# DassHydro-dev/smash

Measured on AMD Instinct MI355X. Metric: cell-timesteps/s, forward+adjoint sweep, higher is better.
Workload: dtype f32

## Files before the change

smash_amd/csrc/smashx.hip:

```cpp
#include "../../include/smashx.h"

#include <hip/hip_runtime.h>
#include <rccl/rccl.h>

#include <dlfcn.h>

#include <algorithm>
#include <cstdio>
#include <cstdlib>
#include <cstring>
#include <string>
#include <vector>

#include "sx_cost.h"
#include "sx_jreg.h"
#include "sx_kernels.h"
#include "sx_ensemble.h"
#include "sx_interception.h"
#include "sx_meanforcing.h"
#include "sx_prcpindices.h"
#include "sx_plan.h"
#include "sx_selftest.h"

namespace {
// ... 279 lines not shown
struct PeerSeg { int rank, first, count; };

struct Launch { hipEvent_t a, b; int kind; double cellsteps; };

}

struct smashx_plan {
    smashx_config cfg{};
    SxSchedule sch;
    int n = 0, npad = 0, nt = 0, ng = 0, st = 0;
    long n2 = 0;
    int M = 0;
    int Tc = 0, nchunks = 0;
    bool have_forcing = false, have_options = false, have_qobs = false, uploaded = false;
    bool chunk_ready = false, adj_ready = false;
    smashx_options opt{};
    std::vector<float> wgauge;
    hipStream_t stream = nullptr;
    hipStream_t stream_r = nullptr;
    int Tp = 0;
    bool hi_tape = true;
    int chain_from = 1;
    bool chain_stage = false; SxStageTables stg{}; int stg_blocks = 0, stg_rows_extra = 0; size_t stg_lds = 0;
    size_t vlds_fwd = 0, vlds_adj = 0;
    std::vector<hipEvent_t> buf_free;
    std::vector<double> round_ncells;
    bool chain_used = false;
    bool chain = true;
    int n_out = 0, n_in = 0;
    int *d_out_x = nullptr, *d_in_x = nullptr;
    float *halo_out = nullptr, *halo_in = nullptr;
    smashx_halo_fn halo_fn = nullptr; void* halo_user = nullptr;
    SxComm* xcomm = nullptr;
    std::vector<PeerSeg> out_segs, in_segs;
    int *d_out_xp = nullptr, *d_in_xp = nullptr;
    float *x_out = nullptr, *x_in = nullptr;
    float* x_keep = nullptr; size_t x_keep_cap = 0;
    std::vector<void*> allocs; std::vector<size_t> alloc_bytes;
    double bytes = 0;
    double hbm_free_at_plan = -1.0, hbm_total = -1.0;
    SxDeviceArrays A{};
    int* d_cell_flat = nullptr;
    int* d_sparse_idx = nullptr;
    float last_jobs_d = 0.f, last_jreg_d = 0.f;
    long n_sparse = 0;
    float* d_stage = nullptr;
// ... 94 lines not shown
    hipStream_t cur = nullptr;
    void mark_begin(int kind, hipStream_t st, double cellsteps = 0.0) {
        cur = st; Launch l; l.a = event(); l.b = nullptr; l.kind = kind; l.cellsteps = cellsteps;
        if (l.a) (void)hipEventRecord(l.a, st);
        launches.push_back(l);
    }
    void mark_end() { Launch& l = launches.back(); l.b = event(); if (l.b) (void)hipEventRecord(l.b, cur); }
};

namespace {

int set_device(const smashx_plan* p) {
    if (p->cfg.device >= 0) HIPCHK(hipSetDevice(p->cfg.device));
    return 0;
}

int sublevels_env() {
    const char* e = getenv("SMASHX_SUBLEVELS");
    const char* e0 = getenv("SMASHX_SUBLEVELS_R0");
    return (e ? std::max(1, atoi(e)) : 1) | ((e0 ? std::max(1, atoi(e0)) : 1) << 8);
}

int chunk_len(const smashx_plan* p, int c) { return std::min(p->Tc, p->nt - c * p->Tc); }

int ensure_chunk_buffers(smashx_plan* p, bool adjoint) {
    const int st = p->st;
    const bool has_hi = (st == 2 || st == 3);
    const double ntape_full = (st == 5 ? 3.0 : st == 3 ? 4.0 : st == 2 ? 3.0 : 2.0);
    const double ntape_lean = has_hi ? ntape_full - 1.0 + 1.0 / SX_HIK : ntape_full;
    double ntape = ntape_full;
    if (!p->chunk_ready) {
        if ((p->n_out > 0 || p->n_in > 0) && p->cfg.chunk_steps <= 0)
            return fail(SMASHX_E_ARG, "a tile with boundary series needs an explicit chunk_steps (identical on every rank; pipe_steps = 0 then means no sub-chunks)");
        const int nt16 = (p->nt + 15) / 16 * 16;
        int Tc = p->cfg.chunk_steps > 0 ? (p->cfg.chunk_steps + 15) / 16 * 16 : 0;
        {
            size_t fr = 0, tot = 0;
            HIPCHK(hipMemGetInfo(&fr, &tot));
            p->hbm_free_at_plan = (double)fr; p->hbm_total = (double)tot;
        }
        if (Tc == 0) {
            size_t fr = 0, tot = 0;
            HIPCHK(hipMemGetInfo(&fr, &tot));
            const double avail = (double)fr * 0.85 - 1.0e9;
            auto fit = [&](double nt_) { return (long)(avail / (4.0 * ((double)p->npad * (2 + nt_) + (double)std::max(p->sch.nxslots, 1)))) / 16 * 16; };
            long t = fit(ntape_full);
            if (has_hi && t < nt16) {
                const long tl = fit(ntape_lean);
                auto nch = [&](long tc) { tc = std::max<long>(16, std::min<long>(nt16, tc)); return (double)((p->nt + tc - 1) / tc); };
                if (0.67 * (1.0 / nch(tl) - 1.0 / nch(t)) > 0.14) { p->hi_tape = false; t = tl; }
            }
            Tc = (int)std::max<long>(16, std::min<long>(nt16, t));
        }
        if (const char* e = getenv("SMASHX_HI_TAPE")) p->hi_tape = atoi(e) != 0;
        if (!has_hi) p->hi_tape = true;
        ntape = p->hi_tape ? ntape_full : ntape_lean;
        (void)ntape;
        Tc = std::min(Tc, nt16);
        {
            const int nch = (p->nt + Tc - 1) / Tc;
            Tc = std::min(Tc, ((p->nt + nch - 1) / nch + 15) / 16 * 16);
        }
        p->Tc = Tc;
        p->A.Tc = Tc;
        p->A.nx = std::max(p->sch.nxslots, 1);
        p->nchunks = (p->nt + Tc - 1) / Tc;
        {
            int want = p->cfg.pipe_steps > 0 ? p->cfg.pipe_steps : Tc;
            const int nsub = std::max(1, (Tc + want / 2) / want);
            p->Tp = std::min(Tc, ((Tc + nsub - 1) / nsub + 15) / 16 * 16);
        }
        int rc;
        if ((rc = p->dmalloc(&p->A.qtT, (size_t)p->npad * Tc))) return rc;
        if ((rc = p->dmalloc(&p->A.xT, (size_t)std::max(p->sch.nxslots, 1) * Tc))) return rc;
        HIPCHK(hipMemsetAsync(p->A.qtT, 0, (size_t)p->npad * Tc * 4, p->stream));
        HIPCHK(hipMemsetAsync(p->A.xT, 0, (size_t)std::max(p->sch.nxslots, 1) * Tc * 4, p->stream));
        p->chunk_ready = true;
    }
    if (p->h_qsim_domain && !p->A.qdT) {
        int rc;
        if ((rc = p->dmalloc(&p->A.qdT, (size_t)p->npad * p->Tc))) return rc;
    }
    if (adjoint && !p->adj_ready) {
        int rc;
        const size_t cs = (size_t)p->npad * p->Tc;
        if (p->A.qsk) { p->dfree(p->A.qsk); p->A.qsk = nullptr; }
        {
            const size_t extra = (size_t)p->sch.max_stage * p->npad * 4;
            const double ntp = 3.0 + ((st == 5 || ((st == 2 || st == 3) && p->hi_tape)) ? 1.0 : (st == 2 || st == 3) ? 1.0 / SX_HIK : 0.0) + (st == 3 ? 1.0 : 0.0);
            size_t fr = 0, tot = 0;
            HIPCHK(hipMemGetInfo(&fr, &tot));
            const double need = 4.0 * ((double)cs * ntp + (double)extra + (double)p->npad * (14 + (p->nchunks > 1 ? 5.0 * p->nchunks : 0.0))
                                       + 2.0 * (double)std::max(p->ngc, 1) * p->nt) + 3.0e9;
            const char* e = getenv("SMASHX_HR_SKEW");
            p->A.hr_skew = (e ? atoi(e) != 0 : true) && (double)fr > need;
            if ((rc = p->dmalloc(&p->A.hrT, cs + (p->A.hr_skew ? extra : 0)))) return rc;
        }
        if ((rc = p->dmalloc(&p->A.tape_hp, cs))) return rc;
        if ((rc = p->dmalloc(&p->A.tape_hft, cs))) return rc;
        if (st == 5 || ((st == 2 || st == 3) && p->hi_tape)) { if ((rc = p->dmalloc(&p->A.tape_hi, cs))) return rc; }
        else if (st == 2 || st == 3) { if ((rc = p->dmalloc(&p->A.ckpt_hi, cs / SX_HIK))) return rc; }
        if (st == 3) { if ((rc = p->dmalloc(&p->A.tape_hst, cs))) return rc; }
        if (p->nchunks > 1) { if ((rc = p->dmalloc(&p->ckpt, (size_t)p->nchunks * 5 * p->npad))) return rc; }
        float** g[14] = {&p->A.ci_b, &p->A.cp_b, &p->A.cft_b, &p->A.cst_b, &p->A.exc_b, &p->A.lr_b,
                         &p->A.hi_b, &p->A.hp_b, &p->A.hft_b, &p->A.hst_b, &p->A.hlr_b, &p->A.px_b[0], &p->A.px_b[1], &p->A.px_b[2]};
        for (auto q : g) if ((rc = p->dmalloc(q, (size_t)p->npad))) return rc;
        if ((rc = p->dmalloc(&p->A.qgb, (size_t)std::max(p->ngc, 1) * p->nt))) return rc;
        if ((rc = p->dmalloc(&p->d_qsim_b, (size_t)std::max(p->ng, 1) * p->nt))) return rc;
        p->adj_ready = true;
    }
    if (p->A.ncs > 0 && !p->A.qsk) {
        const size_t need = (size_t)p->A.ncs * 16 * ((size_t)p->Tc / 4 + p->stg_rows_extra + 1);
        size_t fr = 0, tot = 0;
        HIPCHK(hipMemGetInfo(&fr, &tot));
        if ((double)fr > (double)need + 2.0e9) { int rc; if ((rc = p->dmalloc(&p->A.qsk, need / 4))) return rc; }
    }
    return 0;
}

SxDeviceArrays view_at(const smashx_plan* p, int off) {
    SxDeviceArrays B = p->A;
    B.k0 = 0; B.k1 = p->n;
    const size_t q = (size_t)(off / 4);
    B.qtT = p->A.qtT + q * p->npad * 4;
    if (p->A.hrT) B.hrT = p->A.hrT + q * p->npad * 4;
    if (p->A.qdT) B.qdT = p->A.qdT + q * p->npad * 4;
    if (!p->chain) B.qsk = nullptr;
    B.xT = p->A.xT + q * p->A.nx * 4;
    if (p->A.qtdT) B.qtdT = p->A.qtdT + q * p->npad * 4;
    if (p->A.xdT) B.xdT = p->A.xdT + q * p->A.nx * 4;
    if (p->A.tape_hp) B.tape_hp = p->A.tape_hp + (size_t)off * p->npad;
    if (p->A.tape_hft) B.tape_hft = p->A.tape_hft + (size_t)off * p->npad;
    if (p->A.tape_hi) B.tape_hi = p->A.tape_hi + (size_t)off * p->npad;
    if (p->A.ckpt_hi) B.ckpt_hi = p->A.ckpt_hi + (size_t)(off / SX_HIK) * p->npad;
    if (p->A.tape_hst) B.tape_hst = p->A.tape_hst + (size_t)off * p->npad;
    return B;
}

template <int ST>
void launch_vert_fwd(smashx_plan* p, const SxDeviceArrays& B, bool tape, int t0, int T) {
    const dim3 grid((B.k1 - B.k0 + SX_VBLOCK - 1) / SX_VBLOCK), block(SX_VBLOCK);
    p->mark_begin(0, p->stream, (double)(B.k1 - B.k0) * T);
    const bool cf = B.prcp16 != nullptr;
    const size_t vl = p->vlds_fwd;
    if (tape) { if (cf) hipLaunchKernelGGL((sx_k_vert_fwd<ST, true, true>), grid, block, vl, p->stream, B, t0, T);
                else    hipLaunchKernelGGL((sx_k_vert_fwd<ST, true, false>), grid, block, vl, p->stream, B, t0, T); }
    else      { if (cf) hipLaunchKernelGGL((sx_k_vert_fwd<ST, false, true>), grid, block, vl, p->stream, B, t0, T);
                else    hipLaunchKernelGGL((sx_k_vert_fwd<ST, false, false>), grid, block, vl, p->stream, B, t0, T); }
// ... 48 lines not shown
    return c;
}
int chain_first(const smashx_plan* p) {
    const int nr = p->sch.nrounds;
    return (p->chain && nr - p->chain_from >= 2) ? p->chain_from : nr;
}
void reset_chain_counters(smashx_plan* p, hipStream_t st) {
    (void)hipMemsetAsync(p->A.prog, 0, (size_t)p->sch.ngroups * sizeof(int), st);
    (void)hipMemsetAsync(p->A.prog + p->sch.ngroups + 1, 0, sizeof(int), st);
}
void route_fwd_rounds(smashx_plan* p, int off, bool tape, int t0, int T, hipStream_t st) {
    SxDeviceArrays B = view_at(p, off);
    if (!p->dom_q_active) B.qdT = nullptr;
    const size_t lds = (size_t)2 * p->M * sizeof(float4);
    const int cf = chain_first(p);
    for (int r = 0; r < cf; ++r) {
        const int g0 = p->sch.round_group_begin[r], ngr = p->sch.round_group_begin[r + 1] - g0;
        p->mark_begin(1, st, round_cells(p, r, r + 1) * T);
        if (tape) hipLaunchKernelGGL((sx_k_route_fwd<true, false>), dim3(ngr), dim3(p->M), lds, st, B, g0, g0 + ngr, t0, T);
        else      hipLaunchKernelGGL((sx_k_route_fwd<false, false>), dim3(ngr), dim3(p->M), lds, st, B, g0, g0 + ngr, t0, T);
        p->mark_end();
    }
}
bool route_fwd_chained(smashx_plan* p, int off, bool tape, int t0, int T, hipStream_t st, hipEvent_t inputs_read = nullptr) {
    const int nr = p->sch.nrounds, cf = chain_first(p);
    if (cf >= nr) return false;
    SxDeviceArrays B = view_at(p, off);
    if (!p->dom_q_active) B.qdT = nullptr;
    const size_t lds = (size_t)2 * p->M * sizeof(float4);
    const int g0 = p->sch.round_group_begin[cf], g1 = p->sch.ngroups;
    reset_chain_counters(p, st);
    const int grid = g1 - g0;
    p->mark_begin(5, st, round_cells(p, cf, nr) * T);
    if (B.qsk)
        hipLaunchKernelGGL((sx_k_chain_transpose<true>), dim3((p->stg_blocks + SX_STG_WAVES - 1) / SX_STG_WAVES), dim3(64 * SX_STG_WAVES), p->stg_lds * SX_STG_WAVES, st, B, p->stg, g0, (T + SX_BT - 1) / SX_BT, p->stg_blocks, (int)p->stg_lds);
    const bool early = B.qsk && inputs_read && !B.qdT;
    if (early) (void)hipEventRecord(inputs_read, st);
    if (tape) hipLaunchKernelGGL((sx_k_route_fwd<true, true>), dim3(grid), dim3(p->M), lds, st, B, g0, g1, t0, T);
    else      hipLaunchKernelGGL((sx_k_route_fwd<false, true>), dim3(grid), dim3(p->M), lds, st, B, g0, g1, t0, T);
    p->mark_end();
    p->chain_used = true;
    return early;
}
bool route_fwd(smashx_plan* p, int off, bool tape, int t0, int T, hipEvent_t inputs_read = nullptr) {
    route_fwd_rounds(p, off, tape, t0, T, p->stream_r);
    return route_fwd_chained(p, off, tape, t0, T, p->stream_r, inputs_read);
}
void route_adj_chained(smashx_plan* p, int off, int t0, int T, hipStream_t st) {
    const int nr = p->sch.nrounds, cf = chain_first(p);
    if (cf >= nr) return;
    const SxDeviceArrays B = view_at(p, off);
    const size_t lds = (size_t)2 * p->M * sizeof(float4);
    const int g0 = p->sch.round_group_begin[cf], g1 = p->sch.ngroups;
    reset_chain_counters(p, st);
    const int grid = g1 - g0;
    p->mark_begin(6, st, round_cells(p, cf, nr) * T);
    hipLaunchKernelGGL((sx_k_route_adj<true>), dim3(grid), dim3(p->M), lds, st, B, g0, g1, t0, T);
    if (B.qsk)
        hipLaunchKernelGGL((sx_k_chain_transpose<false>), dim3((p->stg_blocks + SX_STG_WAVES - 1) / SX_STG_WAVES), dim3(64 * SX_STG_WAVES), p->stg_lds * SX_STG_WAVES, st, B, p->stg, g0, (T + SX_BT - 1) / SX_BT, p->stg_blocks, (int)p->stg_lds);
    p->mark_end();
    p->chain_used = true;
}
void route_adj_rounds(smashx_plan* p, int off, int t0, int T, hipStream_t st) {
    const SxDeviceArrays B = view_at(p, off);
    const size_t lds = (size_t)2 * p->M * sizeof(float4);
    const int cf = chain_first(p);
    for (int r = cf - 1; r >= 0; --r) {
        const int g0 = p->sch.round_group_begin[r], ngr = p->sch.round_group_begin[r + 1] - g0;
        p->mark_begin(2, st, round_cells(p, r, r + 1) * T);
        hipLaunchKernelGGL((sx_k_route_adj<false>), dim3(ngr), dim3(p->M), lds, st, B, g0, g0 + ngr, t0, T);
        p->mark_end();
    }
}
void route_adj(smashx_plan* p, int off, int t0, int T) {
    route_adj_chained(p, off, t0, T, p->stream_r);
    route_adj_rounds(p, off, t0, T, p->stream_r);
}

SxCostArgs cost_args(smashx_plan* p, float jobs_b) {
    SxCostArgs C{};
    C.ng = p->ng; C.nt = p->nt; C.s0 = p->opt.optimize_start_step - 1; C.njf = p->opt.njf;
    for (int j = 0; j < SX_MAXJF; ++j) { C.jobs_fun[j] = p->opt.jobs_fun[j]; C.wjobs_fun[j] = p->opt.wjobs_fun[j]; }
    C.dt = p->cfg.dt; C.dx = p->cfg.dx;
    C.qg = p->A.qg; C.qgb = p->A.qgb; C.ngc = p->ngc;
    C.gauge_gid = p->d_gauge_gid; C.gauge_flwacc = p->d_gauge_flwacc; C.area = p->d_area; C.wgauge = p->d_wgauge;
    C.qobs = p->d_qobs; C.qsim_b = p->d_qsim_b; C.sums = p->d_sums; C.coef = p->d_coef; C.out = p->d_cost_out;
    C.med = p->d_med; C.med_idx = p->d_med_idx;
    C.nslots = p->med_nslots; C.slot = p->d_med_slot; C.medx = p->d_medx; C.medx_idx = p->d_medx_idx;
    C.jobs_b = jobs_b;
    return C;
}

int run_cost(smashx_plan* p, int adjoint, float cost_b) {
    if (p->ng == 0 && p->med_nslots == 0) return 0;
    SxCostArgs C = cost_args(p, cost_b);
    p->mark_begin(4, p->stream_r);
    if (p->ng > 0) hipLaunchKernelGGL(sx_k_cost_sums, dim3(p->ng), dim3(64), 0, p->stream_r, C);
    if (p->med_nslots > 0) {
        HIPCHK(hipMemsetAsync(p->d_medx, 0, (size_t)p->med_nslots * sizeof(float), p->stream_r));
// ... 719 lines not shown
    const int ns_max = nsub_of(p->Tc);
    const size_t keep_sub = (size_t)std::max(p->n_in, 1) * (size_t)((p->Tp + 3) / 4) * 4;
    const bool keep_in = adjoint && halo && p->n_in > 0 && C > 1;
    if (keep_in && p->x_keep_cap < keep_sub * ns_max * (size_t)(C - 1)) {
        if (p->x_keep) p->dfree(p->x_keep);
        p->x_keep = nullptr; p->x_keep_cap = 0;
        if ((rc = p->dmalloc(&p->x_keep, keep_sub * ns_max * (size_t)(C - 1)))) return rc;
        p->x_keep_cap = keep_sub * ns_max * (size_t)(C - 1);
    }
    auto inlet_series = [&](int c, int jb, int off, int t0, int T, bool recompute, hipStream_t st) -> int {
        float* msg = native ? p->x_in : p->halo_in;
        float* kept = (keep_in && c < C - 1) ? p->x_keep + ((size_t)c * ns_max + jb) * keep_sub : nullptr;
        const size_t bytes = (size_t)p->n_in * (size_t)((T + 3) / 4) * 4 * sizeof(float);
        if (recompute && kept) {
            HIPCHK(hipMemcpyAsync(msg, kept, bytes, hipMemcpyDeviceToDevice, st));
        } else {
            if ((rc = hook(0, t0, T, st))) return rc;
            if (kept) HIPCHK(hipMemcpyAsync(kept, msg, bytes, hipMemcpyDeviceToDevice, st));
        }
        halo_move(false, false, off, T, st);
        return 0;
    };
    static const bool early_release = []() { const char* e = getenv("SMASHX_EARLY_RELEASE"); return !(e && e[0] == '0'); }();
    auto forward_chunk = [&](int c, bool tape, bool recompute = false) -> int {
        const int t0c = c * p->Tc, Tcur = chunk_len(p, c), ns = nsub_of(Tcur);
        std::vector<hipEvent_t> ev(ns);
        auto launch_v = [&](int jb) -> int {
            const int off = jb * p->Tp, T = std::min(p->Tp, Tcur - off);
            if (jb < (int)p->buf_free.size() && p->buf_free[jb]) { HIPCHK(hipStreamWaitEvent(sV, p->buf_free[jb], 0)); p->buf_free[jb] = nullptr; }
            vert_fwd(p, off, tape, t0c + off, T);
            ev[jb] = p->event(); HIPCHK(hipEventRecord(ev[jb], sV));
            return 0;
        };
        for (int jb = 0; jb < ns; ++jb) if ((rc = launch_v(jb))) return rc;
        for (int jb = 0; jb < ns; ++jb) {
            const int off = jb * p->Tp, T = std::min(p->Tp, Tcur - off);
            if (halo && p->n_in > 0 && (rc = inlet_series(c, jb, off, t0c + off, T, recompute, sR))) return rc;
            HIPCHK(hipStreamWaitEvent(sR, ev[jb], 0));
            if ((int)p->buf_free.size() <= jb) p->buf_free.resize(jb + 1, nullptr);
            p->buf_free[jb] = p->event();
            const bool released = route_fwd(p, off, tape, t0c + off, T, early_release ? p->buf_free[jb] : nullptr);
            if (halo && p->n_out > 0 && !recompute) {
                halo_move(true, true, off, T, sR);
                if ((rc = hook(1, t0c + off, T, sR))) return rc;
            }
            if (!released) HIPCHK(hipEventRecord(p->buf_free[jb], sR));
        }
        return 0;
    };
    p->dom_q_active = !adjoint && p->h_qsim_domain && p->A.qdT;
    auto export_domain = [&](int c) -> int {
        const int t0c = c * p->Tc, Tcur = chunk_len(p, c);
        HIPCHK(hipStreamSynchronize(sV));
        HIPCHK(hipStreamSynchronize(sR));
        const long plane = p->dom_sparse ? p->n_sparse : p->n2;
        const int* idx = p->dom_sparse ? p->d_sparse_idx : p->d_cell_flat;
        const int nbmax = (int)std::max<long>(1, std::min<long>(p->stage_planes * p->n2 / plane, 1 << 15));
        for (int which = 0; which < 2; ++which) {
            float* host = which ? p->h_net_prcp_domain : p->h_qsim_domain;
            const float* src = which ? p->A.qtT : p->A.qdT;
            if (!host || !src) continue;
            for (int tl0 = 0; tl0 < Tcur; tl0 += nbmax) {
                const int nb = std::min(nbmax, Tcur - tl0);
                if (!p->dom_sparse || p->tiled)
// ... 22 lines not shown
            }
            if ((rc = forward_chunk(c, c == C - 1))) return rc;
        }
        if ((rc = run_cost(p, 1, cost_b))) return rc;
        {
            float* gv[14] = {p->A.ci_b, p->A.cp_b, p->A.cft_b, p->A.cst_b, p->A.exc_b, p->A.hi_b, p->A.hp_b, p->A.hft_b, p->A.hst_b,
                             p->A.lr_b, p->A.hlr_b, p->A.px_b[0], p->A.px_b[1], p->A.px_b[2]};
            const int ps = p->st;
            auto pfi = [&](int slot) { const int f = param_field(ps, slot); return f; };
            auto sfi = [&](int slot) { const int f = state_field(ps, slot); return f < 0 ? -1 : SMASHX_GNP + f; };
            const int gi[14] = {pfi(0), pfi(1), pfi(2), pfi(3), pfi(4), sfi(0), sfi(1), sfi(2), sfi(3), pfi(5), sfi(4), pfi(6), pfi(7), pfi(8)};
            bool waited[2] = {false, false};
            for (int q = 0; q < 14; ++q) {
                const bool on_r = (q == 9 || q == 10);
                hipStream_t sq = on_r ? sR : sV;
                HIPCHK(hipMemsetAsync(gv[q], 0, (size_t)p->npad * 4, sq));
                if (p->opt.njr > 0 && gi[q] >= 0 && jreg_optim(p, gi[q]) > 0) {
                    if (!waited[on_r ? 1 : 0]) { HIPCHK(hipStreamWaitEvent(sq, p->ev_j, 0)); waited[on_r ? 1 : 0] = true; }
                    hipLaunchKernelGGL(k_gather, dim3((p->n + 255) / 256), dim3(256), 0, sq, gv[q], p->d_jg[gi[q]], p->d_cell_flat, p->n);
                }
            }
        }
        if (p->ng == 0) HIPCHK(hipMemsetAsync(p->A.qgb, 0, (size_t)std::max(p->ngc, 1) * p->nt * 4, sR));
        for (int c = C - 1; c >= 0; --c) {
            const int t0c = c * p->Tc, Tcur = chunk_len(p, c);
            if (C > 1 && c < C - 1) {
                float* src[5];
                for (int i = 0; i < 5; ++i) src[i] = p->ckpt + ((size_t)c * 5 + i) * p->npad;
                if ((rc = restore_states(p, src))) return rc;
                if ((rc = forward_chunk(c, true, true))) return rc;
            }
            const int nsa = (Tcur + p->Tp - 1) / p->Tp;
            for (int jb = nsa - 1; jb >= 0; --jb) {
                const int off = jb * p->Tp, T = std::min(p->Tp, Tcur - off);
                if (halo && p->n_out > 0) {
                    if ((rc = hook(2, t0c + off, T, sR))) return rc;
                    halo_move(false, true, off, T, sR);
                }
                route_adj(p, off, t0c + off, T);
                hipEvent_t e = p->event();
                HIPCHK(hipEventRecord(e, sR));
                HIPCHK(hipStreamWaitEvent(sV, e, 0));
                vert_adj(p, off, t0c + off, T);
                if (halo && p->n_in > 0) {
                    halo_move(true, false, off, T, sR);
                    if ((rc = hook(3, t0c + off, T, sR))) return rc;
                }
            }
        }
    }
    {
        hipEvent_t e = p->event();
        HIPCHK(hipEventRecord(e, sR));
        HIPCHK(hipStreamWaitEvent(sV, e, 0));
    }
    HIPCHK(hipEventRecord(p->ev1, sV));
    HIPCHK(hipStreamSynchronize(sV));
    HIPCHK(hipStreamSynchronize(sR));
    if (p->opt.njr > 0) HIPCHK(hipStreamSynchronize(p->stream_j));
    HIPCHK(hipGetLastError());
    if (p->chain_used) {
        int stalled = 0;
        HIPCHK(hipMemcpy(&stalled, p->A.prog + p->sch.ngroups, sizeof(int), hipMemcpyDeviceToHost));
        if (stalled) {
            if (getenv("SMASHX_VERBOSE")) {
// ... 4 lines not shown
                std::vector<int> pr(p->sch.ngroups);
                (void)hipMemcpy(pr.data(), p->A.prog, pr.size() * sizeof(int), hipMemcpyDeviceToHost);
                for (int g = p->sch.round_group_begin[chain_first(p)]; g < p->sch.ngroups; ++g) fprintf(stderr, " %d", pr[g]);
                fprintf(stderr, " (n_in %d n_out %d)\n", p->n_in, p->n_out);
            }
            *stalled_out = true; return 0;
        }
    }
    smashx_timing& tm = p->timing;
    std::memset(&tm, 0, sizeof(tm));
    (void)hipEventElapsedTime(&tm.sweep_ms, p->ev0, p->ev1);
    for (const Launch& l : p->launches) {
        float ms = 0.f;
        if (l.a && l.b) (void)hipEventElapsedTime(&ms, l.a, l.b);
        switch (l.kind) {
            case 0: tm.vert_fwd_ms += ms; tm.vert_fwd_launches++; tm.cellsteps[0] += l.cellsteps; break;
            case 1: tm.route_fwd_ms += ms; tm.route_fwd_launches++; tm.cellsteps[1] += l.cellsteps; break;
            case 2: tm.route_adj_ms += ms; tm.route_adj_launches++; tm.cellsteps[2] += l.cellsteps; break;
            case 3: tm.vert_adj_ms += ms; tm.vert_adj_launches++; tm.cellsteps[3] += l.cellsteps; break;
            case 5: tm.route_fwd_ms += ms; tm.route_fwd_launches++; tm.cellsteps[1] += l.cellsteps;
                    tm.route_fwd_chained_ms += ms; tm.route_fwd_chained_launches++; break;
            case 6: tm.route_adj_ms += ms; tm.route_adj_launches++; tm.cellsteps[2] += l.cellsteps;
                    tm.route_adj_chained_ms += ms; tm.route_adj_chained_launches++; break;
            default: tm.cost_ms += ms; break;
        }
    }
    tm.n_chunks = p->nchunks; tm.chunk_steps = p->Tc; tm.pipe_steps = p->Tp; tm.n_rounds = p->sch.nrounds; tm.n_groups = p->sch.ngroups;
    tm.device_bytes = p->bytes;
    tm.max_stage = p->sch.max_stage;
    tm.chain_staged = (p->chain && p->A.qsk != nullptr) ? 1 : 0;
    tm.n_chained_groups = chain_first(p) < p->sch.nrounds ? p->sch.ngroups - p->sch.round_group_begin[chain_first(p)] : 0;
    p->last_adjoint = adjoint;
    return 0;
}

int smashx_set_domain_outputs(smashx_plan* p, float* qsim_domain, float* net_prcp_domain, int sparse) {
    if (!p) return fail(SMASHX_E_ARG, "null plan");
    if (sparse && !p->d_sparse_idx && (qsim_domain || net_prcp_domain))
        return fail(SMASHX_E_ARG, "sparse domain outputs need mesh.path (the sparse cell numbering)");
    p->h_qsim_domain = qsim_domain; p->h_net_prcp_domain = net_prcp_domain; p->dom_sparse = sparse ? 1 : 0;
    return 0;
}

int smashx_debug_group_times(smashx_plan* p, long long* out, int* round_of_group) {
    if (!p || !out) return fail(SMASHX_E_ARG, "null argument");
    if (!p->A.gtime) return fail(SMASHX_E_STATE, "group tracing is off (SMASHX_TRACE_GROUPS=1)");
// ... 1189 lines not shown
```

smash_amd/csrc/sx_kernels.h:

```cpp
#pragma once

#include <hip/hip_runtime.h>

#include <climits>

#include "sx_ops.h"
#include "sx_tangent.h"
#include "sx_vic.h"

#define SX_BT 4
#define SX_VBLOCK 256

__device__ __forceinline__ void sx_lds_barrier() {
    __builtin_amdgcn_fence(__ATOMIC_RELEASE, "workgroup", "local");
    __builtin_amdgcn_s_barrier();
    __builtin_amdgcn_fence(__ATOMIC_ACQUIRE, "workgroup", "local");
}

__device__ __forceinline__ void sx_lds_wave_fence() {
    __builtin_amdgcn_fence(__ATOMIC_RELEASE, "workgroup", "local");
    __builtin_amdgcn_wave_barrier();
    __builtin_amdgcn_fence(__ATOMIC_ACQUIRE, "workgroup", "local");
}

// ... 84 lines not shown
    __builtin_amdgcn_fence(__ATOMIC_ACQUIRE, "agent");
}
__device__ __forceinline__ void sx_publish(int* prog, int blocks) {
    __builtin_amdgcn_fence(__ATOMIC_RELEASE, "agent");
    __hip_atomic_store((sx_gint*)prog, blocks, __ATOMIC_RELAXED, __HIP_MEMORY_SCOPE_AGENT);
}

struct SxDeviceArrays {
    int n, npad, nt, Tc;
    int k0, k1;
    int nx;
    float dt, dx;
    const float* prcp; const float* pet;
    const unsigned short* prcp16; const float* petd; const float* pet_ratio;
    float prcp_c, prcp_gap; int hour0;
    float *ci, *cp, *cft, *cst, *exc, *lr;
    float* px[3]; float* px_b[3];
    float *rt_a, *rt_f, *rt_denf, *rt_denb;
    int* flwacc;
    float *hi, *hp, *hft, *hst, *hlr;
    float *ci_b, *cp_b, *cft_b, *cst_b, *exc_b, *lr_b, *hi_b, *hp_b, *hft_b, *hst_b, *hlr_b;
    float *qtT, *hrT;
    int hr_skew;
    float *qtdT, *xdT, *qgd;
    float* qdT;
    float *tape_hi, *tape_hp, *tape_hft, *tape_hst;
    float* ckpt_hi;
    float* xT;
    float* qsk; int cs0, ncs;
    float *qg, *qgb;
    int* cell_gauge;
    const int *g_slot_begin, *g_dmax;
    const int *s_cell, *s_stage, *s_sub, *s_wsub, *s_child, *s_ccount, *s_parent, *s_xout;
    const int *x_prod, *x_cons;
    int* prog;
    int ngroups;
    int spin_limit;
    int mute_group;
    long long* gtime;
};

struct SxStageTables {
    const int* wb_slot0; const int* wb_n; const int* wb_smin; const int* wb_spread;
    const int* fifo_g; const int* fifo_s;
};
#ifndef SX_STG_PF
// ... 436 lines not shown
            cell = c;
            const int4 cw = reinterpret_cast<const int4*>(A.s_child)[sb + j];
            ch01 = (unsigned)cw.x; ch23 = (unsigned)cw.y; ch45 = (unsigned)cw.z; ch67 = (unsigned)cw.w;
            ccount = A.s_ccount[sb + j]; xout = A.s_xout[sb + j];
            a = A.rt_a[c]; f = A.rt_f[c]; den = (TAN || DFORM) ? A.rt_denb[c] : A.rt_denf[c]; hlr = TAN ? A.hlr_b[c] : A.hlr[c];
            if (TAN) { const float lrv = A.lr[c]; ad = a * ((A.dt / (60.f * lrv)) * A.lr_b[c] / lrv); }
            hasup = A.flwacc[c] > 1;
            gid = A.cell_gauge[c];
        } else {
            xin = -1 - c;
        }
    }
    const float dt = A.dt, dx = A.dx;
    const SxDiv dden = sx_mkdiv(den), ddt = sx_mkdiv(dt);
    const int* wprog = nullptr;
    int seen = 0;
    if (CHAIN && xin >= 0) { const int pg = A.x_prod[xin]; if (pg >= g0 && pg < gend) wprog = A.prog + pg; }
    const bool staged = CHAIN && !TAN && A.qsk != nullptr && valid && !wprog;
    const float4* src = staged ? reinterpret_cast<const float4*>(A.qsk) + (size_t)stage * A.ncs + (sb + j - A.cs0)
                      : (cell >= 0) ? reinterpret_cast<const float4*>(TAN ? A.qtdT : A.qtT) + cell
                                    : reinterpret_cast<const float4*>(TAN ? A.xdT : A.xT) + (xin >= 0 ? xin : 0);
    const size_t sstride = staged ? (size_t)A.ncs : (cell >= 0) ? (size_t)A.npad : (size_t)A.nx;
    float4* x4 = reinterpret_cast<float4*>(TAN ? A.xdT : A.xT);
    float4* hr4 = reinterpret_cast<float4*>(A.hrT);
    const int hs = A.hr_skew ? stage : 0;
    float* gauge_out = TAN ? A.qgd : A.qg;
    const float4 zero4 = make_float4(0.f, 0.f, 0.f, 0.f);
    auto fetch = [&](int tb) -> float4 { return cell >= 0 ? sx_gload4s(src + (size_t)tb * sstride) : sx_gload4(src + (size_t)tb * sstride); };

    float4 nxt[MU], outq[MU], outh[MU], nhr[MU];
    if (CHAIN && wprog) sx_wait_prog(wprog, min(MU - stage, nb), seen, SX_PROG_STALL(A), A.spin_limit, g);
#pragma unroll
    for (int u = 0; u < MU; ++u) {
        const int tb = u - stage;
        nxt[u] = (valid && tb >= 0 && tb < nb) ? fetch(tb) : zero4;
        nhr[u] = (TAN && valid && cell >= 0 && tb >= 0 && tb < nb) ? sx_gload4(hr4 + (size_t)(tb + hs) * A.npad + cell) : zero4;
        outq[u] = zero4; outh[u] = zero4;
    }
    const int nsuper = nb + dmax;
    const int nmacro = (nsuper + MU - 1) / MU;
    for (int mw = 0; mw <= nmacro; ++mw) {
        float4 cur[MU], chr[MU];
#pragma unroll
        for (int u = 0; u < MU; ++u) { cur[u] = nxt[u]; sx_pin(cur[u]); if (TAN) { chr[u] = nhr[u]; sx_pin(chr[u]); } }
        if (CHAIN) asm volatile("s_waitcnt vmcnt(0)" ::: "memory");
        if (mw > 0 && cell >= 0) {
#pragma unroll
            for (int u = 0; u < MU; ++u) {
                const int tb = MU * (mw - 1) + u - stage;
                if (tb >= 0 && tb < nb) {
                    if (xout >= 0) x4[(size_t)tb * A.nx + xout] = outq[u];
                    if (TAPE) sx_gstore4s(hr4 + (size_t)(tb + hs) * A.npad + cell, outh[u]);
                    if (A.qdT) reinterpret_cast<float4*>(A.qdT)[(size_t)tb * A.npad + cell] = outq[u];
                    if (gid >= 0) {
                        const float qv[4] = {outq[u].x, outq[u].y, outq[u].z, outq[u].w};
#pragma unroll
                        for (int i = 0; i < SX_BT; ++i)
                            if (tb * SX_BT + i < T) gauge_out[(size_t)gid * A.nt + t0 + tb * SX_BT + i] = qv[i];
                    }
                }
            }
        }
        if (mw == nmacro) break;
        if (CHAIN && wprog) sx_wait_prog(wprog, min(MU * (mw + 2) - stage, nb), seen, SX_PROG_STALL(A), A.spin_limit, g);
#pragma unroll
        for (int u = 0; u < MU; ++u) {
            const int tb = MU * (mw + 1) + u - stage;
            nxt[u] = (valid && tb >= 0 && tb < nb) ? fetch(tb) : zero4;
            if (TAN) nhr[u] = (valid && cell >= 0 && tb >= 0 && tb < nb) ? sx_gload4(hr4 + (size_t)(tb + hs) * A.npad + cell) : zero4;
        }
#pragma unroll
        for (int u = 0; u < MU; ++u) {
            const int w = MU * mw + u;
            const int tb = w - stage;
            const bool act = valid && tb >= 0 && tb < nb;
            float4* pub = sx_lds + (size_t)(w & 1) * M;
            auto child_val = [&](unsigned e) -> float4 {
                const float4* row = sx_lds + (size_t)((w + 1 + (int)((e >> 15) & 1u)) & 1) * M;
                return row[min((int)(e & 0x7fffu), M - 1)];
            };
          auto sub_pass = [&](const int sl) {
            if (act && sub == sl) {
                const int tl = tb * SX_BT;
                if (cell >= 0) {
                    float s[SX_BT];
                    {
                        const float4 v0 = child_val(ch01 & 0xffffu), v1 = child_val(ch01 >> 16);
                        const bool h0 = ccount > 0, h1 = ccount > 1;
                        s[0] = (h0 ? v0.x : 0.f) + (h1 ? v1.x : 0.f); s[1] = (h0 ? v0.y : 0.f) + (h1 ? v1.y : 0.f);
                        s[2] = (h0 ? v0.z : 0.f) + (h1 ? v1.z : 0.f); s[3] = (h0 ? v0.w : 0.f) + (h1 ? v1.w : 0.f);
                    }
                    for (int c = 2; c < ccount; ++c) {
                        const unsigned wd = c < 4 ? ch23 : c < 6 ? ch45 : ch67;
// ... 97 lines not shown
    bool hasup = false;
    const int nsubw = __builtin_amdgcn_readfirstlane(m > 0 ? A.s_wsub[sb + min(j, m - 1)] : 1);
    if (valid && A.s_cell[sb + j] == INT_MIN) valid = false;
    if (valid) {
        const int c = A.s_cell[sb + j];
        rstage = dmax - A.s_stage[sb + j];
        sub = A.s_sub[sb + j];
        par = A.s_parent[sb + j];
        if (par >= 0) { psame = (par & 0x40000000) != 0; par &= 0xffff; }
        if (c >= 0) {
            cell = c;
            xout = A.s_xout[sb + j];
            a = A.rt_a[c]; f = A.rt_f[c]; den = A.rt_denb[c]; lr = A.lr[c];
            hr_b = A.hlr_b[c]; lr_b = A.lr_b[c];
            hasup = A.flwacc[c] > 1;
            gid = A.cell_gauge[c];
        } else {
            xin = -1 - c;
        }
    }
    const float dt = A.dt, dx = A.dx;
    const SxDiv dden = sx_mkdiv(den), ddt = sx_mkdiv(dt), dlr = sx_mkdiv((lr * lr) * 60.f);
    float4* x4 = reinterpret_cast<float4*>(A.xT);
    const float4* hr4p = reinterpret_cast<const float4*>(A.hrT);
    const int hs = A.hr_skew ? dmax - rstage : 0;
    float4* qt4 = reinterpret_cast<float4*>(A.qtT);
    const float4 zero4 = make_float4(0.f, 0.f, 0.f, 0.f);
    const bool root_in = (cell >= 0 && par < 0 && xout >= 0);
    const bool staged = CHAIN && A.qsk != nullptr && valid && (cell >= 0 || (xin >= 0 && !(A.x_prod[xin] >= g0 && A.x_prod[xin] < gend)));
    float4* const dst = staged ? reinterpret_cast<float4*>(A.qsk) + (size_t)(dmax - rstage) * A.ncs + (sb + j - A.cs0)
                               : (cell >= 0) ? qt4 + cell : x4 + (xin >= 0 ? xin : 0);
    const size_t dstride = staged ? (size_t)A.ncs : (cell >= 0) ? (size_t)A.npad : (size_t)A.nx;

    const float* seedp = (gid >= 0) ? A.qgb + (size_t)gid * A.nt + t0 : nullptr;
    auto load_seed = [&](int tb) -> float4 {
        float4 v = make_float4(0.f, 0.f, 0.f, 0.f);
        if (gid >= 0) {
            const int tl = tb * SX_BT;
            if (tl + 0 < T) v.x = sx_gload1(seedp + tl + 0);
            if (tl + 1 < T) v.y = sx_gload1(seedp + tl + 1);
            if (tl + 2 < T) v.z = sx_gload1(seedp + tl + 2);
            if (tl + 3 < T) v.w = sx_gload1(seedp + tl + 3);
        }
        return v;
    };
    const int* wprog = nullptr;
    int seen = 0;
    if (CHAIN && root_in) { const int cg = A.x_cons[xout]; if (cg >= g0 && cg < gend) wprog = A.prog + cg; }
    auto fetch_in = [&](int tb) -> float4 { return sx_gload4(x4 + (size_t)tb * A.nx + xout); };
    float4 nhr[MU], nin[MU], nsd[MU], outq[MU];
    if (CHAIN && wprog) sx_wait_prog(wprog, min(MU - rstage, nb), seen, SX_PROG_STALL(A), A.spin_limit, g);
#pragma unroll
    for (int u = 0; u < MU; ++u) {
        const int tbr = u - rstage;
        const int tb = nb - 1 - tbr;
        const bool ok = valid && tbr >= 0 && tbr < nb;
        nhr[u] = (ok && cell >= 0) ? sx_gload4s(hr4p + (size_t)(tb + hs) * A.npad + cell) : zero4;
        nin[u] = (ok && root_in) ? fetch_in(tb) : zero4;
        nsd[u] = ok ? load_seed(tb) : zero4;
        outq[u] = zero4;
    }
    const int nsuper = nb + dmax;
    const int nmacro = (nsuper + MU - 1) / MU;
    for (int mw = 0; mw <= nmacro; ++mw) {
        float4 chr[MU], cin[MU], csd[MU];
#pragma unroll
        for (int u = 0; u < MU; ++u) {
            chr[u] = nhr[u]; cin[u] = nin[u]; csd[u] = nsd[u];
            sx_pin(chr[u]); sx_pin(cin[u]); sx_pin(csd[u]);
        }
        if (CHAIN) asm volatile("s_waitcnt vmcnt(0)" ::: "memory");
        if (mw > 0 && valid) {
#pragma unroll
            for (int u = 0; u < MU; ++u) {
                const int tbr = MU * (mw - 1) + u - rstage;
                if (tbr >= 0 && tbr < nb) {
                    const int tb = nb - 1 - tbr;
                    sx_gstore4(dst + (size_t)tb * dstride, outq[u]);
                }
            }
        }
        if (mw == nmacro) break;
        if (CHAIN && wprog) sx_wait_prog(wprog, min(MU * (mw + 2) - rstage, nb), seen, SX_PROG_STALL(A), A.spin_limit, g);
#pragma unroll
        for (int u = 0; u < MU; ++u) {
            const int tbr = MU * (mw + 1) + u - rstage;
            const int tb = nb - 1 - tbr;
            const bool ok = valid && tbr >= 0 && tbr < nb;
            nhr[u] = (ok && cell >= 0) ? sx_gload4s(hr4p + (size_t)(tb + hs) * A.npad + cell) : zero4;
            nin[u] = (ok && root_in) ? fetch_in(tb) : zero4;
            nsd[u] = ok ? load_seed(tb) : zero4;
        }
#pragma unroll
        for (int u = 0; u < MU; ++u) {
            const int w = MU * mw + u;
            const int tbr = w - rstage;
            const bool act = valid && tbr >= 0 && tbr < nb;
            float4* pub = sx_lds + (size_t)(w & 1) * M;
            const float4* prev = sx_lds + (size_t)((w + 1) & 1) * M;
          auto sub_pass = [&](const int sl) {
            if (act && sub == sl) {
                const int tb = nb - 1 - tbr;
                const int tl = tb * SX_BT;
                float4 in4 = cin[u];
                if (par >= 0) in4 = psame ? pub[par] : prev[par];
                if (cell >= 0) {
                    const float hrv[SX_BT] = {chr[u].x, chr[u].y, chr[u].z, chr[u].w};
                    const float inv[SX_BT] = {in4.x, in4.y, in4.z, in4.w};
                    const float sdv[SX_BT] = {csd[u].x, csd[u].y, csd[u].z, csd[u].w};
                    float pb[SX_BT], qtb[SX_BT];
                    float tmpb[SX_BT], qrb[SX_BT], himb[SX_BT], a1b[SX_BT];
                    float nq[SX_BT];
#pragma unroll
                    for (int i = SX_BT - 1; i >= 0; --i) {
                        float q_b = 0.f;
// ... 157 lines not shown
```

Baseline: 54.80 billion.

## Keep chained routing tape per chunk and overlap next chunk's chained adjoint

Adds a persistent per-chunk buffer (hrk) that stores the chained-routing hr tape for every chunk except the last, so the adjoint sweep no longer recomputes the chained forward routing for those chunks. The skewed hr tape becomes a circular row buffer addressed by wrapped row indices instead of extra padded rows, which removes the free-memory check and the extra allocation. The chained adjoint for the previous chunk is also launched early on the routing stream so it overlaps with the vertical adjoint of the current chunk. In exchange it uses extra device memory proportional to the number of chunks, and it adds wrap-around index arithmetic inside the forward and adjoint routing kernels.

Result: faster. 57.68 billion, median of 6 (+5.2%).

```diff
diff --git a/smash_amd/csrc/smashx.hip b/smash_amd/csrc/smashx.hip
--- a/smash_amd/csrc/smashx.hip
+++ b/smash_amd/csrc/smashx.hip
@@ -325,6 +325,7 @@
     bool hi_tape = true;
     int chain_from = 1;
     bool chain_stage = false; SxStageTables stg{}; int stg_blocks = 0, stg_rows_extra = 0; size_t stg_lds = 0;
+    float* hrk = nullptr; bool hrk_tried = false, early_adj = true;
     size_t vlds_fwd = 0, vlds_adj = 0;
     std::vector<hipEvent_t> buf_free;
     std::vector<double> round_ncells;
@@ -465,6 +466,7 @@
 }
 
 int chunk_len(const smashx_plan* p, int c) { return std::min(p->Tc, p->nt - c * p->Tc); }
+int chain_first(const smashx_plan* p);
 
 int ensure_chunk_buffers(smashx_plan* p, bool adjoint) {
     const int st = p->st;
@@ -506,6 +508,7 @@
         }
         p->Tc = Tc;
         p->A.Tc = Tc;
+        p->A.hr_rows = Tc / 4;
         p->A.nx = std::max(p->sch.nxslots, 1);
         p->nchunks = (p->nt + Tc - 1) / Tc;
         {
@@ -529,15 +532,9 @@
         const size_t cs = (size_t)p->npad * p->Tc;
         if (p->A.qsk) { p->dfree(p->A.qsk); p->A.qsk = nullptr; }
         {
-            const size_t extra = (size_t)p->sch.max_stage * p->npad * 4;
-            const double ntp = 3.0 + ((st == 5 || ((st == 2 || st == 3) && p->hi_tape)) ? 1.0 : (st == 2 || st == 3) ? 1.0 / SX_HIK : 0.0) + (st == 3 ? 1.0 : 0.0);
-            size_t fr = 0, tot = 0;
-            HIPCHK(hipMemGetInfo(&fr, &tot));
-            const double need = 4.0 * ((double)cs * ntp + (double)extra + (double)p->npad * (14 + (p->nchunks > 1 ? 5.0 * p->nchunks : 0.0))
-                                       + 2.0 * (double)std::max(p->ngc, 1) * p->nt) + 3.0e9;
             const char* e = getenv("SMASHX_HR_SKEW");
-            p->A.hr_skew = (e ? atoi(e) != 0 : true) && (double)fr > need;
-            if ((rc = p->dmalloc(&p->A.hrT, cs + (p->A.hr_skew ? extra : 0)))) return rc;
+            p->A.hr_skew = e ? atoi(e) != 0 : true;
+            if ((rc = p->dmalloc(&p->A.hrT, cs))) return rc;
         }
         if ((rc = p->dmalloc(&p->A.tape_hp, cs))) return rc;
         if ((rc = p->dmalloc(&p->A.tape_hft, cs))) return rc;
@@ -558,6 +555,23 @@
         HIPCHK(hipMemGetInfo(&fr, &tot));
         if ((double)fr > (double)need + 2.0e9) { int rc; if ((rc = p->dmalloc(&p->A.qsk, need / 4))) return rc; }
     }
+    if (adjoint && !p->hrk_tried) {
+        p->hrk_tried = true;
+        const int cf = chain_first(p);
+        const char* e = getenv("SMASHX_KEEP_CHAIN_TAPE");
+        const bool want = e ? atoi(e) != 0 : true;
+        if (const char* ea = getenv("SMASHX_EARLY_ADJ_CHAIN")) p->early_adj = atoi(ea) != 0;
+        if (want && p->nchunks > 1 && cf < p->sch.nrounds && !p->tiled && p->n_in == 0 && p->n_out == 0 && p->Tp >= p->Tc) {
+            const int kcs0 = p->sch.g_slot_begin[p->sch.round_group_begin[cf]], kncs = p->sch.nslots - kcs0;
+            const size_t need = (size_t)(p->nchunks - 1) * (size_t)(p->Tc / 4) * (size_t)kncs * 16;
+            size_t fr = 0, tot = 0;
+            HIPCHK(hipMemGetInfo(&fr, &tot));
+            if (kncs > 0 && (double)fr > (double)need + 2.0e9) {
+                int rc; if ((rc = p->dmalloc(&p->hrk, need / 4))) return rc;
+                p->A.kcs0 = kcs0; p->A.kncs = kncs;
+            }
+        }
+    }
     return 0;
 }
 
@@ -566,7 +580,8 @@
     B.k0 = 0; B.k1 = p->n;
     const size_t q = (size_t)(off / 4);
     B.qtT = p->A.qtT + q * p->npad * 4;
-    if (p->A.hrT) B.hrT = p->A.hrT + q * p->npad * 4;
+    B.hrk = nullptr;
+    if (p->A.hrT) { if (p->A.hr_skew) B.hr_row0 = (int)q; else B.hrT = p->A.hrT + q * p->npad * 4; }
     if (p->A.qdT) B.qdT = p->A.qdT + q * p->npad * 4;
     if (!p->chain) B.qsk = nullptr;
     B.xT = p->A.xT + q * p->A.nx * 4;
@@ -661,10 +676,11 @@
         p->mark_end();
     }
 }
-bool route_fwd_chained(smashx_plan* p, int off, bool tape, int t0, int T, hipStream_t st, hipEvent_t inputs_read = nullptr) {
+bool route_fwd_chained(smashx_plan* p, int off, bool tape, int t0, int T, hipStream_t st, hipEvent_t inputs_read = nullptr, float* hrk = nullptr) {
     const int nr = p->sch.nrounds, cf = chain_first(p);
     if (cf >= nr) return false;
     SxDeviceArrays B = view_at(p, off);
+    if (hrk) { B.hrk = hrk; B.hr_row0 = 0; tape = true; }
     if (!p->dom_q_active) B.qdT = nullptr;
     const size_t lds = (size_t)2 * p->M * sizeof(float4);
     const int g0 = p->sch.round_group_begin[cf], g1 = p->sch.ngroups;
@@ -681,24 +697,26 @@
     p->chain_used = true;
     return early;
 }
-bool route_fwd(smashx_plan* p, int off, bool tape, int t0, int T, hipEvent_t inputs_read = nullptr) {
-    route_fwd_rounds(p, off, tape, t0, T, p->stream_r);
-    return route_fwd_chained(p, off, tape, t0, T, p->stream_r, inputs_read);
-}
-void route_adj_chained(smashx_plan* p, int off, int t0, int T, hipStream_t st) {
+void route_adj_chained(smashx_plan* p, int off, int t0, int T, hipStream_t st, float* hrk = nullptr, bool launch = true, bool copy = true) {
     const int nr = p->sch.nrounds, cf = chain_first(p);
     if (cf >= nr) return;
-    const SxDeviceArrays B = view_at(p, off);
+    SxDeviceArrays B = view_at(p, off);
+    if (hrk) { B.hrk = hrk; B.hr_row0 = 0; }
     const size_t lds = (size_t)2 * p->M * sizeof(float4);
     const int g0 = p->sch.round_group_begin[cf], g1 = p->sch.ngroups;
-    reset_chain_counters(p, st);
     const int grid = g1 - g0;
-    p->mark_begin(6, st, round_cells(p, cf, nr) * T);
-    hipLaunchKernelGGL((sx_k_route_adj<true>), dim3(grid), dim3(p->M), lds, st, B, g0, g1, t0, T);
-    if (B.qsk)
+    if (launch) {
+        reset_chain_counters(p, st);
+        p->mark_begin(6, st, round_cells(p, cf, nr) * T);
+        hipLaunchKernelGGL((sx_k_route_adj<true>), dim3(grid), dim3(p->M), lds, st, B, g0, g1, t0, T);
+        p->mark_end();
+        p->chain_used = true;
+    }
+    if (copy && B.qsk) {
+        p->mark_begin(7, st);
         hipLaunchKernelGGL((sx_k_chain_transpose<false>), dim3((p->stg_blocks + SX_STG_WAVES - 1) / SX_STG_WAVES), dim3(64 * SX_STG_WAVES), p->stg_lds * SX_STG_WAVES, st, B, p->stg, g0, (T + SX_BT - 1) / SX_BT, p->stg_blocks, (int)p->stg_lds);
-    p->mark_end();
-    p->chain_used = true;
+        p->mark_end();
+    }
 }
 void route_adj_rounds(smashx_plan* p, int off, int t0, int T, hipStream_t st) {
     const SxDeviceArrays B = view_at(p, off);
@@ -710,10 +728,6 @@
         hipLaunchKernelGGL((sx_k_route_adj<false>), dim3(ngr), dim3(p->M), lds, st, B, g0, g0 + ngr, t0, T);
         p->mark_end();
     }
-}
-void route_adj(smashx_plan* p, int off, int t0, int T) {
-    route_adj_chained(p, off, t0, T, p->stream_r);
-    route_adj_rounds(p, off, t0, T, p->stream_r);
 }
 
 SxCostArgs cost_args(smashx_plan* p, float jobs_b) {
@@ -1479,6 +1493,8 @@
         return 0;
     };
     static const bool early_release = []() { const char* e = getenv("SMASHX_EARLY_RELEASE"); return !(e && e[0] == '0'); }();
+    const bool keep = adjoint && C > 1 && p->hrk && !halo && chain_first(p) < p->sch.nrounds;
+    auto kept_rows = [&](int c) -> float* { return (keep && c < C - 1) ? p->hrk + (size_t)c * (size_t)(p->Tc / 4) * (size_t)p->A.kncs * 4 : nullptr; };
     auto forward_chunk = [&](int c, bool tape, bool recompute = false) -> int {
         const int t0c = c * p->Tc, Tcur = chunk_len(p, c), ns = nsub_of(Tcur);
         std::vector<hipEvent_t> ev(ns);
@@ -1496,7 +1512,9 @@
             HIPCHK(hipStreamWaitEvent(sR, ev[jb], 0));
             if ((int)p->buf_free.size() <= jb) p->buf_free.resize(jb + 1, nullptr);
             p->buf_free[jb] = p->event();
-            const bool released = route_fwd(p, off, tape, t0c + off, T, early_release ? p->buf_free[jb] : nullptr);
+            float* const hrk = kept_rows(c);
+            route_fwd_rounds(p, off, tape, t0c + off, T, sR);
+            const bool released = (hrk && recompute) ? false : route_fwd_chained(p, off, tape, t0c + off, T, sR, early_release ? p->buf_free[jb] : nullptr, hrk);
             if (halo && p->n_out > 0 && !recompute) {
                 halo_move(true, true, off, T, sR);
                 if ((rc = hook(1, t0c + off, T, sR))) return rc;
@@ -1565,6 +1583,7 @@
             }
         }
         if (p->ng == 0) HIPCHK(hipMemsetAsync(p->A.qgb, 0, (size_t)std::max(p->ngc, 1) * p->nt * 4, sR));
+        bool adj_queued = false;
         for (int c = C - 1; c >= 0; --c) {
             const int t0c = c * p->Tc, Tcur = chunk_len(p, c);
             if (C > 1 && c < C - 1) {
@@ -1580,10 +1599,16 @@
                     if ((rc = hook(2, t0c + off, T, sR))) return rc;
                     halo_move(false, true, off, T, sR);
                 }
-                route_adj(p, off, t0c + off, T);
+                route_adj_chained(p, off, t0c + off, T, sR, kept_rows(c), !adj_queued, true);
+                adj_queued = false;
+                route_adj_rounds(p, off, t0c + off, T, sR);
                 hipEvent_t e = p->event();
                 HIPCHK(hipEventRecord(e, sR));
                 HIPCHK(hipStreamWaitEvent(sV, e, 0));
+                if (jb == 0 && c > 0 && kept_rows(c - 1) && p->early_adj && p->chain && p->A.qsk) {
+                    route_adj_chained(p, 0, (c - 1) * p->Tc, chunk_len(p, c - 1), sR, kept_rows(c - 1), true, false);
+                    adj_queued = true;
+                }
                 vert_adj(p, off, t0c + off, T);
                 if (halo && p->n_in > 0) {
                     halo_move(true, false, off, T, sR);
@@ -1634,6 +1659,7 @@
                     tm.route_fwd_chained_ms += ms; tm.route_fwd_chained_launches++; break;
             case 6: tm.route_adj_ms += ms; tm.route_adj_launches++; tm.cellsteps[2] += l.cellsteps;
                     tm.route_adj_chained_ms += ms; tm.route_adj_chained_launches++; break;
+            case 7: tm.route_adj_ms += ms; tm.route_adj_chained_ms += ms; break;
             default: tm.cost_ms += ms; break;
         }
     }
diff --git a/smash_amd/csrc/sx_kernels.h b/smash_amd/csrc/sx_kernels.h
--- a/smash_amd/csrc/sx_kernels.h
+++ b/smash_amd/csrc/sx_kernels.h
@@ -130,6 +130,8 @@
     float *ci_b, *cp_b, *cft_b, *cst_b, *exc_b, *lr_b, *hi_b, *hp_b, *hft_b, *hst_b, *hlr_b;
     float *qtT, *hrT;
     int hr_skew;
+    int hr_rows, hr_row0;
+    float* hrk; int kcs0, kncs;
     float *qtdT, *xdT, *qgd;
     float* qdT;
     float *tape_hi, *tape_hp, *tape_hft, *tape_hst;
@@ -612,8 +614,15 @@
                                     : reinterpret_cast<const float4*>(TAN ? A.xdT : A.xT) + (xin >= 0 ? xin : 0);
     const size_t sstride = staged ? (size_t)A.ncs : (cell >= 0) ? (size_t)A.npad : (size_t)A.nx;
     float4* x4 = reinterpret_cast<float4*>(TAN ? A.xdT : A.xT);
-    float4* hr4 = reinterpret_cast<float4*>(A.hrT);
-    const int hs = A.hr_skew ? stage : 0;
+    const bool kept = CHAIN && TAPE && !TAN && A.hrk != nullptr;
+    const bool circ = A.hr_skew || kept;
+    float4* const hr4 = kept ? reinterpret_cast<float4*>(A.hrk) + (sb + j - A.kcs0) : reinterpret_cast<float4*>(A.hrT) + max(cell, 0);
+    const size_t hstride = kept ? (size_t)A.kncs : (size_t)A.npad;
+    const int hrows = A.hr_rows;
+    static_assert(SX_MU_F <= 4, "the row wrap assumes a macro-step no longer than the shortest chunk (16 steps = 4 rows)");
+    auto hwrap = [&](int r) { return r >= hrows ? r - hrows : r; };
+    auto hrow = [&](int base, int u, int tb) { return circ ? hwrap(base + u) : tb; };
+    int hrw_prev = 0, hrw = circ ? A.hr_row0 : 0;
     float* gauge_out = TAN ? A.qgd : A.qg;
     const float4 zero4 = make_float4(0.f, 0.f, 0.f, 0.f);
     auto fetch = [&](int tb) -> float4 { return cell >= 0 ? sx_gload4s(src + (size_t)tb * sstride) : sx_gload4(src + (size_t)tb * sstride); };
@@ -624,7 +633,7 @@
     for (int u = 0; u < MU; ++u) {
         const int tb = u - stage;
         nxt[u] = (valid && tb >= 0 && tb < nb) ? fetch(tb) : zero4;
-        nhr[u] = (TAN && valid && cell >= 0 && tb >= 0 && tb < nb) ? sx_gload4(hr4 + (size_t)(tb + hs) * A.npad + cell) : zero4;
+        nhr[u] = (TAN && valid && cell >= 0 && tb >= 0 && tb < nb) ? sx_gload4(hr4 + (size_t)hrow(hrw, u, tb) * hstride) : zero4;
         outq[u] = zero4; outh[u] = zero4;
     }
     const int nsuper = nb + dmax;
@@ -640,7 +649,7 @@
                 const int tb = MU * (mw - 1) + u - stage;
                 if (tb >= 0 && tb < nb) {
                     if (xout >= 0) x4[(size_t)tb * A.nx + xout] = outq[u];
-                    if (TAPE) sx_gstore4s(hr4 + (size_t)(tb + hs) * A.npad + cell, outh[u]);
+                    if (TAPE) sx_gstore4s(hr4 + (size_t)hrow(hrw_prev, u, tb) * hstride, outh[u]);
                     if (A.qdT) reinterpret_cast<float4*>(A.qdT)[(size_t)tb * A.npad + cell] = outq[u];
                     if (gid >= 0) {
                         const float qv[4] = {outq[u].x, outq[u].y, outq[u].z, outq[u].w};
@@ -657,8 +666,9 @@
         for (int u = 0; u < MU; ++u) {
             const int tb = MU * (mw + 1) + u - stage;
             nxt[u] = (valid && tb >= 0 && tb < nb) ? fetch(tb) : zero4;
-            if (TAN) nhr[u] = (valid && cell >= 0 && tb >= 0 && tb < nb) ? sx_gload4(hr4 + (size_t)(tb + hs) * A.npad + cell) : zero4;
-        }
+            if (TAN) nhr[u] = (valid && cell >= 0 && tb >= 0 && tb < nb) ? sx_gload4(hr4 + (size_t)hrow(hwrap(hrw + MU), u, tb) * hstride) : zero4;
+        }
+        hrw_prev = hrw; hrw = hwrap(hrw + MU);
 #pragma unroll
         for (int u = 0; u < MU; ++u) {
             const int w = MU * mw + u;
@@ -802,8 +812,15 @@
     const float dt = A.dt, dx = A.dx;
     const SxDiv dden = sx_mkdiv(den), ddt = sx_mkdiv(dt), dlr = sx_mkdiv((lr * lr) * 60.f);
     float4* x4 = reinterpret_cast<float4*>(A.xT);
-    const float4* hr4p = reinterpret_cast<const float4*>(A.hrT);
-    const int hs = A.hr_skew ? dmax - rstage : 0;
+    const bool kept = CHAIN && A.hrk != nullptr;
+    const bool circ = A.hr_skew || kept;
+    const float4* const hr4p = kept ? reinterpret_cast<const float4*>(A.hrk) + (sb + j - A.kcs0) : reinterpret_cast<const float4*>(A.hrT) + max(cell, 0);
+    const size_t hstride = kept ? (size_t)A.kncs : (size_t)A.npad;
+    const int hrows = A.hr_rows;
+    static_assert(SX_MU_A <= 4, "the row wrap assumes a macro-step no longer than the shortest chunk (16 steps = 4 rows)");
+    auto hwrap = [&](int r) { return r < 0 ? r + hrows : r; };
+    auto hrow = [&](int base, int u, int tb) { return circ ? hwrap(base - u) : tb; };
+    int hrw = circ ? (A.hr_row0 + nb - 1 + dmax) % hrows : 0;
     float4* qt4 = reinterpret_cast<float4*>(A.qtT);
     const float4 zero4 = make_float4(0.f, 0.f, 0.f, 0.f);
     const bool root_in = (cell >= 0 && par < 0 && xout >= 0);
@@ -835,11 +852,12 @@
         const int tbr = u - rstage;
         const int tb = nb - 1 - tbr;
         const bool ok = valid && tbr >= 0 && tbr < nb;
-        nhr[u] = (ok && cell >= 0) ? sx_gload4s(hr4p + (size_t)(tb + hs) * A.npad + cell) : zero4;
+        nhr[u] = (ok && cell >= 0) ? sx_gload4s(hr4p + (size_t)hrow(hrw, u, tb) * hstride) : zero4;
         nin[u] = (ok && root_in) ? fetch_in(tb) : zero4;
         nsd[u] = ok ? load_seed(tb) : zero4;
         outq[u] = zero4;
     }
+    hrw = hwrap(hrw - MU);
     const int nsuper = nb + dmax;
     const int nmacro = (nsuper + MU - 1) / MU;
     for (int mw = 0; mw <= nmacro; ++mw) {
@@ -867,10 +885,11 @@
             const int tbr = MU * (mw + 1) + u - rstage;
             const int tb = nb - 1 - tbr;
             const bool ok = valid && tbr >= 0 && tbr < nb;
-            nhr[u] = (ok && cell >= 0) ? sx_gload4s(hr4p + (size_t)(tb + hs) * A.npad + cell) : zero4;
+            nhr[u] = (ok && cell >= 0) ? sx_gload4s(hr4p + (size_t)hrow(hrw, u, tb) * hstride) : zero4;
             nin[u] = (ok && root_in) ? fetch_in(tb) : zero4;
             nsd[u] = ok ? load_seed(tb) : zero4;
         }
+        hrw = hwrap(hrw - MU);
 #pragma unroll
         for (int u = 0; u < MU; ++u) {
             const int w = MU * mw + u;
```
